# ZeayW/Multimodal-fusion-based-Pre-routing-Timing-Prediction-

Measured on AMD Instinct MI355X. Metric: train-step samples/sec, higher is better.
Workload: dtype bf16; 1 GPU; config B: 8 designs/step/GPU, 65536-node netlist, 64 levels, 256x256 tile, 1350 endpoints/design, UNet(max), bf16 operands / fp32 accumulate on the MFMA-bound contractions; U-Net activations and their gradients stored bf16, netlist tensors, statistics, parameters and gradients fp32; nodes=65536, levels=64, tile=256, endpoints_per_design=1350, cone_pruning=False, parallelism=dp1 (designs sharded, one all-reduce of the flat gradient per step), launch=one HIP graph replay per step (Adam inside)

## Files before the change

### multimodal-fusion-based-pre-routing-timing-prediction-_amd/csrc/linear.hip

```cpp
#include "gemm_engine.h"
#include <string.h>

namespace mmft {

static thread_local char g_err[512] = {0};

void set_error(const char* fmt, ...) {
  va_list ap;
  va_start(ap, fmt);
  vsnprintf(g_err, sizeof(g_err), fmt, ap);
  va_end(ap);
}

static int g_math_mode = 0;
int math_mode() { return __atomic_load_n(&g_math_mode, __ATOMIC_RELAXED); }

}
#include <mutex>
#include <string>
#include <vector>
#include <map>
namespace mmft {
struct ProfRec {
  const char* name;
// ... 256 lines not shown
    float v = x[i];
    if (act == ACT_RELU) v = v > 0.f ? v : 0.f;
    else if (act == ACT_LEAKY) v = v > 0.f ? v : v * slope;
    y[i] = v;
  }
}

__global__ void stamp_kernel(unsigned long long* slots, int index) { slots[index] = wall_clock64(); }

}

using namespace mmft;

extern "C" {

int mmft_version(void) { return 204; }

int mmft_set_math_mode(int mode) {
  MMFT_REQUIRE(mode == MMFT_MATH_F32 || mode == MMFT_MATH_BF16, "set_math_mode: unknown mode %d", mode);
  __atomic_store_n(&mmft::g_math_mode, mode, __ATOMIC_RELAXED);
  return MMFT_OK;
}

int mmft_get_math_mode(void) { return mmft::math_mode(); }

int mmft_prof_enable(int on) {
  std::lock_guard<std::mutex> lk(mmft::g_prof_mu);
  mmft::g_prof = on != 0;
  return MMFT_OK;
}

// ... 212 lines not shown
```

### multimodal-fusion-based-pre-routing-timing-prediction-_amd/csrc/unet16_conv.hip

```cpp
#include <type_traits>
#include "unet16.h"

namespace mmft {

struct U16PackDesc {
  const float* w;
  u16* out;
  int rows, K;
  int taps;
  int mode;
  int Rsrc, Ksrc;
};

__global__ void __launch_bounds__(256) u16_pack_kernel(const U16PackDesc* __restrict__ descs, long long* __restrict__ counters,
                                                       int ncounters, long long inc) {
  if (counters && blockIdx.x == 0 && blockIdx.y == 0 && (int)threadIdx.x < ncounters) counters[threadIdx.x] += inc;
  const U16PackDesc d = descs[blockIdx.y];
  const int mode = d.mode & 3, KW = (d.mode & 4) ? 8 : 4, G = KW / 4;
  const int KB = d.K / (4 * KW), MB = d.rows / 16;
  const long long items = (long long)MB * d.taps * KB * 64 * G;
  for (long long e = (long long)blockIdx.x * 256 + threadIdx.x; e < items; e += (long long)gridDim.x * 256) {
    const int g = (int)(e % G);
    const int lane = (int)((e / G) & 63);
    long long f = e / (64 * G);
// ... 462 lines not shown
  if (!name[0])
    snprintf(name, sizeof(name), EVAL ? "u16_conv3x3_eval_kernel<%d,%d,%dx%d%s>" : "u16_conv3x3_kernel<%d,%d,%dx%d%s>", RGB ? 3 : CI, COB,
             TH, TW, a.stats ? "" : "");
  MMFT_LAUNCH_LDS(name, flops, bytes, (u16_conv3x3_kernel<CI, COB, TH, TW, RGB, EVAL>), dim3(grid_x, a.CO / COB), dim3(256),
                  C::LDS_BYTES, st, a);
  return check_launch(EVAL ? "u16_conv3x3_eval" : "u16_conv3x3");
}

template <bool EVAL>
static int u16_conv_dispatch(U16ConvArgs& a, int rgb_f32, int Ci, hipStream_t st, double flops, double bytes) {
  int th, tw;
  u16_tile_shape(a.W, &th, &tw);
  a.tiles_x = (a.W + tw - 1) / tw;
  a.tiles_y = (a.H + th - 1) / th;
  a.tiles = a.N * a.tiles_x * a.tiles_y;
  const int cob = a.CO % 32 == 0 ? 32 : 16, gy = a.CO / cob;
  int cap = 2048 / gy;
  const int gx = a.tiles < cap ? a.tiles : cap;
#define U16_CONV(CIV, COBV, RGBV)                                                                           \
  (tw == 64 ? u16_conv_launch_t<CIV, COBV, 4, 64, RGBV, EVAL>(a, gx, st, flops, bytes)                      \
            : u16_conv_launch_t<CIV, COBV, 8, 32, RGBV, EVAL>(a, gx, st, flops, bytes))
  if (rgb_f32) return U16_CONV(16, 16, true);
  if (cob == 16) {
    if (Ci == 16) return U16_CONV(16, 16, false);
    if (Ci == 32) return U16_CONV(32, 16, false);
    if (Ci == 64) return U16_CONV(64, 16, false);
    return U16_CONV(128, 16, false);
  }
  if (Ci == 16) return U16_CONV(16, 32, false);
  if (Ci == 32) return U16_CONV(32, 32, false);
  if (Ci == 64) return U16_CONV(64, 32, false);
// ... 142 lines not shown
```

### multimodal-fusion-based-pre-routing-timing-prediction-_amd/csrc/unet16_ew.hip

```cpp
#include "unet16.h"

namespace mmft {

__device__ __forceinline__ double wave_sum_d(double v) {
  for (int o = 32; o > 0; o >>= 1) v += __shfl_xor(v, o, 64);
  return v;
}

__global__ void __launch_bounds__(64) u16_bn_finalize_kernel(const float* __restrict__ stats, int tiles_per_image, int N, int C,
                                                             double count, float eps, const float* __restrict__ gamma,
                                                             const float* __restrict__ beta, float* __restrict__ bnp) {
  const int img = blockIdx.x / C, c = blockIdx.x % C, lane = threadIdx.x;
  const long long NC = (long long)N * C;
  double s = 0.0, ss = 0.0;
  for (int t = lane; t < tiles_per_image; t += 64) {
    const float* p = stats + ((long long)(img * tiles_per_image + t) * 2) * C;
    s += (double)p[c];
    ss += (double)p[C + c];
  }
  s = wave_sum_d(s);
  ss = wave_sum_d(ss);
  if (lane == 0) {
    const double mean = s / count;
    double var = ss / count - mean * mean;
    if (var < 0.0) var = 0.0;
    const float invstd = (float)(1.0 / sqrt(var + (double)eps));
    const float scale = gamma[c] * invstd;
    const long long o = (long long)img * C + c;
    bnp[o] = (float)mean;
    bnp[NC + o] = invstd;
    bnp[2 * NC + o] = (float)var;
    bnp[3 * NC + o] = scale;
    bnp[4 * NC + o] = __fmaf_rn(-(float)mean, scale, beta[c]);
  }
}

struct U16Running {
  float* mean;
  float* var;
  float momentum;
  double count;
};
__device__ __forceinline__ void u16_running_update(const float* __restrict__ bnp, int N, int C, const U16Running& run) {
  const int c = threadIdx.x;
  if (c >= C) return;
  const long long NC = (long long)N * C;
  double rm = (double)run.mean[c], rv = (double)run.var[c];
  for (int img = 0; img < N; ++img) {
    const double var = (double)bnp[2 * NC + (long long)img * C + c];
// ... 5 lines not shown
  run.var[c] = (float)rv;
}

struct U16ApplyArgs {
  const u16* z;
  const float* scale;
  const float* shift;
  u16* a;
  int lda;
  u16* pooled;
  int N, H, W, C, pool_mode;
  const float* bnp;
  U16Running run;
};

__global__ void __launch_bounds__(256) u16_bn_apply_kernel(U16ApplyArgs p) {
  if (p.run.mean && blockIdx.x == 0) u16_running_update(p.bnp, p.N, p.C, p.run);
  const int CG = p.C / 8;
  const long long per_img = (long long)p.H * p.W * CG, total = per_img * p.N;
  for (long long it = (long long)blockIdx.x * 256 + threadIdx.x; it < total; it += (long long)gridDim.x * 256) {
    const int cg = (int)(it % CG);
    const long long pix = it / CG;
    const int img = (int)(it / per_img);
    float sc[8], sh[8], f[8];
    const float* s0 = p.scale + (long long)img * p.C + cg * 8;
    const float* h0 = p.shift + (long long)img * p.C + cg * 8;
    *reinterpret_cast<f32x4*>(sc) = *reinterpret_cast<const f32x4*>(s0);
    *reinterpret_cast<f32x4*>(sc + 4) = *reinterpret_cast<const f32x4*>(s0 + 4);
    *reinterpret_cast<f32x4*>(sh) = *reinterpret_cast<const f32x4*>(h0);
    *reinterpret_cast<f32x4*>(sh + 4) = *reinterpret_cast<const f32x4*>(h0 + 4);
    unpack8(*reinterpret_cast<const u32x4*>(p.z + pix * p.C + cg * 8), f);
#pragma unroll
    for (int j = 0; j < 8; ++j) {
      const float t = bn_pre(f[j], sc[j], sh[j]);
      f[j] = t > 0.f ? t : 0.f;
    }
    *reinterpret_cast<u32x4*>(p.a + pix * p.lda + cg * 8) = pack8(f);
  }
}

__global__ void __launch_bounds__(256) u16_bn_apply_pool_kernel(U16ApplyArgs p) {
  if (p.run.mean && blockIdx.x == 0) u16_running_update(p.bnp, p.N, p.C, p.run);
  const int CG = p.C / 8, H2 = p.H / 2, W2 = p.W / 2;
  const long long per_img = (long long)H2 * W2 * CG, total = per_img * p.N;
  for (long long it = (long long)blockIdx.x * 256 + threadIdx.x; it < total; it += (long long)gridDim.x * 256) {
    const int cg = (int)(it % CG);
    const long long win = it / CG;
    const int x2 = (int)(win % W2), y2 = (int)((win / W2) % H2), img = (int)(win / ((long long)W2 * H2));
    float sc[8], sh[8];
    const float* s0 = p.scale + (long long)img * p.C + cg * 8;
    const float* h0 = p.shift + (long long)img * p.C + cg * 8;
    *reinterpret_cast<f32x4*>(sc) = *reinterpret_cast<const f32x4*>(s0);
    *reinterpret_cast<f32x4*>(sc + 4) = *reinterpret_cast<const f32x4*>(s0 + 4);
    *reinterpret_cast<f32x4*>(sh) = *reinterpret_cast<const f32x4*>(h0);
    *reinterpret_cast<f32x4*>(sh + 4) = *reinterpret_cast<const f32x4*>(h0 + 4);
    const long long p00 = ((long long)img * p.H + 2 * y2) * p.W + 2 * x2;
    u32x4 zv[4];
#pragma unroll
    for (int k = 0; k < 4; ++k)
      zv[k] = *reinterpret_cast<const u32x4*>(p.z + (p00 + (k >> 1) * p.W + (k & 1)) * p.C + cg * 8);
    float best[8];
#pragma unroll
    for (int k = 0; k < 4; ++k) {
      float f[8];
      unpack8(zv[k], f);
#pragma unroll
      for (int j = 0; j < 8; ++j) {
        const float t = bn_pre(f[j], sc[j], sh[j]);
        f[j] = t > 0.f ? t : 0.f;
      }
      const u32x4 av = pack8(f);
      *reinterpret_cast<u32x4*>(p.a + (p00 + (k >> 1) * p.W + (k & 1)) * p.lda + cg * 8) = av;
      unpack8(av, f);
#pragma unroll
      for (int j = 0; j < 8; ++j) {
        if (p.pool_mode == MMFT_POOL_MAX) best[j] = (k == 0 || f[j] > best[j] || f[j] != f[j]) ? f[j] : best[j];
        else best[j] = k == 0 ? f[j] : best[j] + f[j];
      }
    }
    if (p.pool_mode != MMFT_POOL_MAX) {
#pragma unroll
      for (int j = 0; j < 8; ++j) best[j] *= 0.25f;
    }
    *reinterpret_cast<u32x4*>(p.pooled + (((long long)img * H2 + y2) * W2 + x2) * p.C + cg * 8) = pack8(best);
  }
}

__global__ void __launch_bounds__(256) u16_bn_bwd_partial_kernel(const u16* __restrict__ g, const u16* __restrict__ z,
                                                                 const float* __restrict__ bnp, long long rows, int N, int C,
                                                                 int blocks_per_image, float* __restrict__ partial) {
  __shared__ float red[2][256 * 8];
  const int img = blockIdx.x / blocks_per_image, blk = blockIdx.x % blocks_per_image;
  const long long NC = (long long)N * C;
  const long long rpb = (rows + blocks_per_image - 1) / blocks_per_image;
  const long long r0 = (long long)blk * rpb, r1 = r0 + rpb < rows ? r0 + rpb : rows;
  const int CG = C / 8;
  const int rstep = 256 / CG;
  const int cg = threadIdx.x % CG, rl = threadIdx.x / CG;
  float s[8], sx[8];
// ... 91 lines not shown
    const int cg = (int)(it % CG);
    const long long pix = it / CG;
    const int img = (int)(it / per_img);
    const long long o = (long long)img * C + cg * 8, e = pix * C + cg * 8;
    float gv[8], zf[8], out[8];
    unpack8(*reinterpret_cast<const u32x4*>(g + e), gv);
    unpack8(*reinterpret_cast<const u32x4*>(z + e), zf);
#pragma unroll
    for (int j = 0; j < 8; ++j) {
      const float mu = bnp[o + j], is = bnp[NC + o + j], sc = bnp[3 * NC + o + j], sh = bnp[4 * NC + o + j];
      const float gm = bn_pre(zf[j], sc, sh) > 0.f ? gv[j] : 0.f;
      const float xh = (zf[j] - mu) * is;
      out[j] = sc * (gm - coef[o + j] - xh * coef[NC + o + j]);
    }
    *reinterpret_cast<u32x4*>(dz + e) = pack8(out);
  }
}

struct U16PoolBwdArgs {
  const u16* a;
  int lda;
  const u16* gskip;
  int ldg;
  const u16* gp;
  u16* g;
  int N, H, W, C, pool_mode;
};

__global__ void __launch_bounds__(256) u16_pool_bwd_kernel(U16PoolBwdArgs p) {
  const int CG = p.C / 8, H2 = p.H / 2, W2 = p.W / 2;
// ... 68 lines not shown
  MMFT_REQUIRE(!running_mean == !running_var, "u16_bn_apply: running_mean and running_var come together");
  MMFT_REQUIRE(aligned16(z) && aligned16(a) && aligned16(bnp) && (!pooled || aligned16(pooled)), "u16_bn_apply: 16-byte alignment");
  DeviceGuard dg(device);
  const long long NC = (long long)N * C;
  U16ApplyArgs p{reinterpret_cast<const u16*>(z), bnp + 3 * NC, bnp + 4 * NC, reinterpret_cast<u16*>(a), lda,
                 reinterpret_cast<u16*>(pooled), N, H, W, C, pool_mode, bnp, U16Running{running_mean, running_var, momentum, (double)H * W}};
  const double by = 2.0 * N * H * W * C * (pooled ? 2.25 : 2.0);
  if (pooled) {
    const long long items = (long long)N * (H / 2) * (W / 2) * (C / 8);
    MMFT_LAUNCH("u16_bn_apply_pool_kernel", 0.0, by, u16_bn_apply_pool_kernel, dim3(ew_grid(items)), dim3(256), (hipStream_t)stream, p);
  } else {
    const long long items = (long long)N * H * W * (C / 8);
    MMFT_LAUNCH("u16_bn_apply_kernel", 0.0, by, u16_bn_apply_kernel, dim3(ew_grid(items)), dim3(256), (hipStream_t)stream, p);
  }
  return check_launch("u16_bn_apply");
}

long long mmft_u16_bn_bwd_workspace_bytes(int N, long long pixels_per_image, int C) {
  return (long long)N * u16_bwd_blocks(pixels_per_image) * 2 * C * 4 + (long long)2 * N * C * 4;
}

int mmft_u16_bn_bwd(const void* g, const void* z, const float* bnp, void* dz, float* dgamma, float* dbeta, int accumulate, int N,
                    long long pixels_per_image, int C, float* workspace, long long workspace_bytes, int device, void* stream) {
  MMFT_REQUIRE(g && z && bnp && dz && dgamma && dbeta && N > 0 && pixels_per_image > 0 && C >= 8 && C % 8 == 0 && C <= 128,
               "u16_bn_bwd: bad arguments (C a multiple of 8, <= 128)");
  MMFT_REQUIRE(workspace && workspace_bytes >= mmft_u16_bn_bwd_workspace_bytes(N, pixels_per_image, C), "u16_bn_bwd: workspace too small");
  MMFT_REQUIRE(aligned16(g) && aligned16(z) && aligned16(dz), "u16_bn_bwd: 16-byte alignment");
  DeviceGuard dg(device);
  hipStream_t st = (hipStream_t)stream;
  const int bpi = u16_bwd_blocks(pixels_per_image);
// ... 2 lines not shown
  const double elems = (double)N * pixels_per_image * C;
  MMFT_LAUNCH("u16_bn_bwd_partial_kernel", 0.0, 4.0 * elems, u16_bn_bwd_partial_kernel, dim3(N * bpi), dim3(256), st,
              reinterpret_cast<const u16*>(g), reinterpret_cast<const u16*>(z), bnp, pixels_per_image, N, C, bpi, partial);
  int rc = check_launch("u16_bn_bwd_partial");
  if (rc) return rc;
  MMFT_LAUNCH("u16_bn_bwd_finalize_kernel", 0.0, 8.0 * N * bpi * C, u16_bn_bwd_finalize_kernel, dim3(C), dim3(256), st, partial, bpi, N, C,
              (double)pixels_per_image, coef, dgamma, dbeta, accumulate ? 1 : 0);
  rc = check_launch("u16_bn_bwd_finalize");
  if (rc) return rc;
  const long long items = (long long)N * pixels_per_image * (C / 8);
  MMFT_LAUNCH("u16_bn_bwd_apply_kernel", 0.0, 6.0 * elems, u16_bn_bwd_apply_kernel, dim3(ew_grid(items)), dim3(256), st,
              reinterpret_cast<const u16*>(g), reinterpret_cast<const u16*>(z), bnp, coef, reinterpret_cast<u16*>(dz), pixels_per_image, N, C);
  return check_launch("u16_bn_bwd_apply");
}

int mmft_u16_pool_bwd(const void* a, int lda, const void* gskip, int ldg, const void* gp, void* g, int N, int H, int W, int C,
                      int pool_mode, int device, void* stream) {
  MMFT_REQUIRE(a && gp && g && N > 0 && H > 0 && W > 0 && H % 2 == 0 && W % 2 == 0 && C >= 8 && C % 8 == 0 && lda >= C && lda % 8 == 0 &&
                   (!gskip || (ldg >= C && ldg % 8 == 0)),
               "u16_pool_bwd: bad arguments");
  MMFT_REQUIRE(aligned16(a) && aligned16(gp) && aligned16(g) && (!gskip || aligned16(gskip)), "u16_pool_bwd: 16-byte alignment");
  DeviceGuard dg(device);
  U16PoolBwdArgs p{reinterpret_cast<const u16*>(a), lda, reinterpret_cast<const u16*>(gskip), ldg, reinterpret_cast<const u16*>(gp),
                   reinterpret_cast<u16*>(g), N, H, W, C, pool_mode};
  const long long items = (long long)N * (H / 2) * (W / 2) * (C / 8);
  MMFT_LAUNCH("u16_pool_bwd_kernel", 0.0, 2.0 * N * H * W * C * (gskip ? 3.25 : 2.25), u16_pool_bwd_kernel, dim3(ew_grid(items)), dim3(256),
              (hipStream_t)stream, p);
  return check_launch("u16_pool_bwd");
}

// ... 2 lines not shown
```

### multimodal-fusion-based-pre-routing-timing-prediction-_amd/mmft/lib.py

```python
import contextlib
import ctypes
import os
import re
import threading
import torch

_HERE = os.path.dirname(os.path.abspath(__file__))
PKG_DIR = os.path.dirname(_HERE)
LIB_PATH = os.environ.get('MMFT_LIB') or os.path.join(PKG_DIR, 'lib', 'libmmft_hip.so')
HEADER_PATH = os.path.join(os.path.dirname(PKG_DIR), 'include', 'mmft.h')
EXT_HEADER_PATH = os.path.join(os.path.dirname(PKG_DIR), 'include', 'mmft_report.h')
PLACE_HEADER_PATH = os.path.join(os.path.dirname(PKG_DIR), 'include', 'mmft_place.h')
INCR_HEADER_PATH = os.path.join(os.path.dirname(PKG_DIR), 'include', 'mmft_incr.h')

_lib = None


def _parse_header(path):
    with open(path) as f:
        text = f.read()
    text = re.sub(r'/\*.*?\*/', '', text, flags=re.S)
    decls = {}
    for ret, name, params in re.findall(r'\b(int|long long|const char\*)\s+(mmft_[a-z0-9_]+)\s*\(([^)]*)\)\s*;', text):
        args = []
        params = params.strip()
        if params and params != 'void':
            for prm in params.split(','):
                prm = prm.strip()
# ... 20 lines not shown
    return _parse_header(HEADER_PATH)


def ext_decls():
    return _parse_header(EXT_HEADER_PATH)


def place_decls():
    return _parse_header(PLACE_HEADER_PATH)


def incr_decls():
    return _parse_header(INCR_HEADER_PATH)


def header_symbols():
    return sorted(header_decls())


def load():
    global _lib
    if _lib is None:
        if not os.path.exists(LIB_PATH):
            raise RuntimeError(
                f"libmmft_hip.so not found at {LIB_PATH}; build it with `python __graft_entry__.py build` "
                f"(make -C {os.path.join(PKG_DIR, 'csrc')}). There is no CPU/eager fallback for the hot path.")
        _lib = ctypes.CDLL(LIB_PATH)
        for name, (res, args) in header_decls().items():
            fn = getattr(_lib, name)
            fn.restype = res
# ... 76 lines not shown
    return int(rc)


_INCR = {}


def incr(name, *args):
    fn = _INCR.get(name)
    if fn is None:
        decls = incr_decls()
        if name not in decls:
            raise RuntimeError(f'{name} is not declared in {INCR_HEADER_PATH}')
        fn = getattr(load(), name)
        fn.restype, fn.argtypes = decls[name]
        _INCR[name] = fn
    rc = fn(*[a.data_ptr() if isinstance(a, _Tensor) else a for a in args])
    if rc != 0:
        raise RuntimeError(f"{name} failed ({rc}): {load().mmft_last_error().decode()}")
    return int(rc)


_workspace = {}
_retired = []
_scope = threading.local()


@contextlib.contextmanager
def scratch_owner(owner):
    prev, _scope.owner = getattr(_scope, 'owner', None), owner
    try:
# ... 108 lines not shown
```

### multimodal-fusion-based-pre-routing-timing-prediction-_amd/mmft/unet16.py

```python
import ctypes
import functools
import math
import weakref

import torch
from torch import nn

from . import gradsink, lib, ops

ENABLED = True


def supported(net, x, frozen_stats=False):
    if not ENABLED or net.bilinear or x.dim() != 4 or x.shape[1] != 3 or x.dtype != torch.float32 or not x.is_cuda:
        return False
    if x.shape[0] > 1 and not net.inc.per_sample_stats and not frozen_stats:
        return False
    H, W = x.shape[2], x.shape[3]
    return H % 8 == 0 and W % 32 == 0 and H >= 8


def _params(net):
    ps = net.__dict__.get('_u16_param_list')
    if ps is None:
# ... 162 lines not shown

@functools.lru_cache(maxsize=16)
def _bwd_sizes(N, H, W):
    lv, P = _geometry(N, H, W)
    sizes = [('g%d' % i, P[_CONV[i][2]] * _CONV[i][1]) for i in range(1, 15)] + [('dz%d' % i, P[_CONV[i][2]] * _CONV[i][1]) for i in range(1, 15)]
    sizes += [('gcat3', P[0] * 32), ('gcat2', P[1] * 64), ('gcat1', P[2] * 128), ('gp1', P[1] * 16), ('gp2', P[2] * 32), ('gp3', P[3] * 64)]
    q = lib.query
    ws_bytes = max([q('mmft_u16_outconv_bwd_workspace_bytes', N, H, W)] +
                   [q('mmft_u16_bn_bwd_workspace_bytes', N, lv[_CONV[i][2]][0] * lv[_CONV[i][2]][1], _CONV[i][1]) for i in range(1, 15)] +
                   [q('mmft_u16_conv3x3_wgrad_workspace_bytes', N, lv[_CONV[i][2]][0], lv[_CONV[i][2]][1], _CONV[i][0], _CONV[i][1])
                    for i in range(1, 15)] +
                   [q('mmft_u16_convt_wgrad_workspace_bytes', N, lv[u[4]][0], lv[u[4]][1], u[0]) for u in _UP.values()])
    return sizes, ws_bytes


BATCH_REDUCE = True


@functools.lru_cache(maxsize=16)
def _slab_sizes(N, H, W):
    lv, _ = _geometry(N, H, W)
    q = lib.query
    sizes = [('sw%d' % i, q('mmft_u16_conv3x3_wgrad_workspace_bytes', N, lv[_CONV[i][2]][0], lv[_CONV[i][2]][1], _CONV[i][0], _CONV[i][1]) // 4)
             for i in range(1, 15)]
    sizes += [('st%d' % k, q('mmft_u16_convt_wgrad_workspace_bytes', N, lv[u[4]][0], lv[u[4]][1], u[0]) // 4) for k, u in _UP.items()]
    sizes += [('so', q('mmft_u16_outconv_bwd_workspace_bytes', N, H, W) // 4)]
    return sizes


def _run_forward(net, xn, pool_mode, packs, T, F, out, geom):
    N, H, W = geom
    dev, st = lib.stream_args(out)
    lv, _ = _geometry(N, H, W)
    convs = _layers(net)
    ups = [net.up1.up, net.up2.up, net.up3.up]
    packs.refresh(net, counters=net._batch_counters(), inc=N if net.inc.per_sample_stats else 1)
    per_img = ctypes.c_int(0)
    for i in range(1, 15):
        Ci, Co, l, inp = _CONV[i]
        h, w = lv[l]
        cv, bn = convs[i - 1]
        xin = xn if inp == 'x' else T[inp]
        lib.load().mmft_u16_conv_tiles(N, h, w, ctypes.byref(per_img))
        lib.call('mmft_u16_conv3x3', xin, 1 if inp == 'x' else 0, packs.ptr('f%d' % (i - 1)), T['z%d' % i], F['stats'], N, h, w,
                 Ci, Co, dev, st)
        lib.call('mmft_u16_bn_finalize', F['stats'], per_img.value, N, Co, h * w, float(bn.eps), bn.weight.detach(), bn.bias.detach(),
                 F['bnp%d' % i], dev, st)
        abuf_name, lda, pooled = _ACT[i]
        lib.call('mmft_u16_bn_apply', T['z%d' % i], F['bnp%d' % i], T[abuf_name], lda, T[pooled] if pooled else None, N, h, w, Co,
                 pool_mode, float(bn.momentum), bn.running_mean, bn.running_var, dev, st)
        for k, (uCi, uin, cat, coff, ul) in _UP.items():
            if uin == abuf_name:
                up = ups[k]
                uh, uw = lv[ul]
                lib.call('mmft_u16_convt_fwd', T[uin], packs.ptr('tf%d' % k), up.bias.detach() if up.bias is not None else None,
                         T[cat].data_ptr() + coff * 2, 2 * (uCi // 2), N, uh, uw, uCi, dev, st)
    oc = net.outc.conv[0]
    lib.call('mmft_u16_outconv_fwd', T['a14'], oc.weight.detach(), oc.bias.detach() if oc.bias is not None else None, out, N, H, W,
             pool_mode, dev, st)


@functools.lru_cache(maxsize=16)
def _eval_sizes(N, H, W):
    return [(name, n) for name, n in _fwd_sizes(N, H, W)[0] if not name.startswith('z')]

# ... 82 lines not shown
        so = SL['so']
        lib.call('mmft_u16_outconv_bwd', T['a14'], oc.weight.detach(), oc.bias.detach() if oc.bias is not None else None, g, G['g14'],
                 None, None, 0, N, H, W, pool_mode, so, so.numel() * 4, dev, st)
        ns = lib.query('mmft_u16_outconv_bwd_slabs', N, H, W)
        reduce_later(so.data_ptr(), s_w.out, ns, 17, 16, 1, s_w.accumulate)
        if s_b is not None:
            reduce_later(so.data_ptr() + 64, s_b.out, ns, 17, 1, 1, s_b.accumulate)

    def conv_backward(i):
        Ci, Co, l, inp = _CONV[i]
        h, w = lv[l]
        cv, bn = convs[i - 1]
        s_g, s_bt = sinks[id(bn.weight)], sinks[id(bn.bias)]
        if s_g.accumulate != s_bt.accumulate:
            raise RuntimeError('unet16: BatchNorm weight / bias sinks out of step')
        lib.call('mmft_u16_bn_bwd', G['g%d' % i], T['z%d' % i], F['bnp%d' % i], G['dz%d' % i], s_g.out, s_bt.out, int(s_g.accumulate),
                 N, h * w, Co, ws, ws.numel() * 4, dev, st)
        s_cw = sinks[id(cv.weight)]
        xin = xn if inp == 'x' else T[inp]
        if SL is None:
            lib.call('mmft_u16_conv3x3_wgrad', xin, 1 if inp == 'x' else 0, G['dz%d' % i], s_cw.out, int(s_cw.accumulate), N, h, w, Ci, Co,
                     ws, ws.numel() * 4, dev, st)
        else:
            sw = SL['sw%d' % i]
            lib.call('mmft_u16_conv3x3_wgrad', xin, 1 if inp == 'x' else 0, G['dz%d' % i], None, 0, N, h, w, Ci, Co,
                     sw, sw.numel() * 4, dev, st)
            reduce_later(sw.data_ptr(), s_cw.out, lib.query('mmft_u16_conv3x3_wgrad_slabs', N, h, w, Ci, Co), Co * 9 * Ci, Co * 9 * Ci, 1,
                         s_cw.accumulate)
        if inp == 'x':
            return
        tgt = {'cat1': 'gcat1', 'cat2': 'gcat2', 'cat3': 'gcat3', 'p1': 'gp1', 'p2': 'gp2', 'p3': 'gp3'}.get(inp)
        if tgt is None:
# ... 20 lines not shown
            if s_ub is not None:
                reduce_later(stb.data_ptr() + 4 * wel, s_ub.out, ns, wel + 4 * Co, Co, 4, s_ub.accumulate)
        lib.call('mmft_u16_convt_dgrad', gslice, 2 * Co, packs.ptr('tb%d' % k), G[g_target], N, uh, uw, uCi, dev, st)

    def pool_backward(cat, C, l, gp, g_target):
        h, w = lv[l]
        lib.call('mmft_u16_pool_bwd', T[cat], 2 * C, G['g' + cat], 2 * C, G[gp], G[g_target], N, h, w, C, pool_mode, dev, st)

    conv_backward(14); conv_backward(13); up_backward(2, 'g12')
    conv_backward(12); conv_backward(11); up_backward(1, 'g10')
    conv_backward(10); conv_backward(9); up_backward(0, 'g8')
    conv_backward(8); conv_backward(7); pool_backward('cat1', 64, 2, 'gp3', 'g6')
    conv_backward(6); conv_backward(5); pool_backward('cat2', 32, 1, 'gp2', 'g4')
    conv_backward(4); conv_backward(3); pool_backward('cat3', 16, 0, 'gp1', 'g2')
    conv_backward(2); conv_backward(1)
    if table:
        lib.call('mmft_slab_reduce_batch', torch.tensor(table, dtype=torch.int64), len(table), dev, st)


REPLAY = True


class _Token:
    __slots__ = ('__weakref__',)


class _Replay:

    def __init__(self, key):
        self.key, self.x_ref, self.x_version = key, None, None
        self.fwd, self.bwd = lib.GraphReplay(), lib.GraphReplay()
        self.pending = None
# ... 92 lines not shown
```

Before: 2441 designs/s.

## Fuse BN finalize with apply for small U-Net levels and add fused BN backward

Adds a single-launch kernel that recomputes the per-image BatchNorm coefficients from tile statistics inside each apply block and writes bnp and running stats from block 0. It is used for small spatial levels with at least 64 channels, removing a separate finalize launch and its dependency bubble. It also adds a fused BN backward kernel (disabled by default), switches the conv dispatch to 16-channel output blocks when the 128-input-channel grid is too small, and chunks the slab-reduce batch. The cost is redundant coefficient recomputation per block and some added code paths.

```diff
diff --git a/include/mmft_unet_small.h b/include/mmft_unet_small.h
--- /dev/null
+++ b/include/mmft_unet_small.h
@@ -0,0 +1,19 @@
+#ifndef MMFT_UNET_SMALL_H
+#define MMFT_UNET_SMALL_H
+
+#include "mmft.h"
+
+#ifdef __cplusplus
+extern "C" {
+#endif
+
+int mmft_u16_bn_finalize_apply(const float* stats, int tiles_per_image, int N, int C, long long pixels_per_image, float eps,
+                               const float* gamma, const float* beta, float* bnp, const void* z, void* a, int lda, void* pooled, int H,
+                               int W, int pool_mode, float momentum, float* running_mean, float* running_var, int device, void* stream);
+int mmft_u16_bn_bwd_fused(const void* g, const void* z, const float* bnp, void* dz, float* sums, float* dgamma, float* dbeta,
+                          int accumulate, int N, long long pixels_per_image, int C, int device, void* stream);
+
+#ifdef __cplusplus
+}
+#endif
+#endif
diff --git a/multimodal-fusion-based-pre-routing-timing-prediction-_amd/csrc/linear.hip b/multimodal-fusion-based-pre-routing-timing-prediction-_amd/csrc/linear.hip
--- a/multimodal-fusion-based-pre-routing-timing-prediction-_amd/csrc/linear.hip
+++ b/multimodal-fusion-based-pre-routing-timing-prediction-_amd/csrc/linear.hip
@@ -294,7 +294,7 @@
 
 extern "C" {
 
-int mmft_version(void) { return 204; }
+int mmft_version(void) { return 205; }
 
 int mmft_set_math_mode(int mode) {
   MMFT_REQUIRE(mode == MMFT_MATH_F32 || mode == MMFT_MATH_BF16, "set_math_mode: unknown mode %d", mode);
diff --git a/multimodal-fusion-based-pre-routing-timing-prediction-_amd/csrc/unet16_conv.hip b/multimodal-fusion-based-pre-routing-timing-prediction-_amd/csrc/unet16_conv.hip
--- a/multimodal-fusion-based-pre-routing-timing-prediction-_amd/csrc/unet16_conv.hip
+++ b/multimodal-fusion-based-pre-routing-timing-prediction-_amd/csrc/unet16_conv.hip
@@ -500,7 +500,8 @@
   a.tiles_x = (a.W + tw - 1) / tw;
   a.tiles_y = (a.H + th - 1) / th;
   a.tiles = a.N * a.tiles_x * a.tiles_y;
-  const int cob = a.CO % 32 == 0 ? 32 : 16, gy = a.CO / cob;
+  const bool narrow = Ci == 128 && (long long)a.tiles * (a.CO / 32) < 256;
+  const int cob = (a.CO % 32 == 0 && !narrow) ? 32 : 16, gy = a.CO / cob;
   int cap = 2048 / gy;
   const int gx = a.tiles < cap ? a.tiles : cap;
 #define U16_CONV(CIV, COBV, RGBV)                                                                           \
diff --git a/multimodal-fusion-based-pre-routing-timing-prediction-_amd/csrc/unet16_ew.hip b/multimodal-fusion-based-pre-routing-timing-prediction-_amd/csrc/unet16_ew.hip
--- a/multimodal-fusion-based-pre-routing-timing-prediction-_amd/csrc/unet16_ew.hip
+++ b/multimodal-fusion-based-pre-routing-timing-prediction-_amd/csrc/unet16_ew.hip
@@ -1,10 +1,34 @@
 #include "unet16.h"
+#include "../../include/mmft_unet_small.h"
 
 namespace mmft {
 
 __device__ __forceinline__ double wave_sum_d(double v) {
   for (int o = 32; o > 0; o >>= 1) v += __shfl_xor(v, o, 64);
   return v;
+}
+
+struct U16Coef {
+  float mean, invstd, var, scale, shift;
+};
+__device__ __forceinline__ U16Coef u16_bn_coef(double s, double ss, double count, float eps, float gamma, float beta) {
+  const double mean = s / count;
+  double var = ss / count - mean * mean;
+  if (var < 0.0) var = 0.0;
+  U16Coef k;
+  k.invstd = (float)(1.0 / sqrt(var + (double)eps));
+  k.scale = gamma * k.invstd;
+  k.mean = (float)mean;
+  k.var = (float)var;
+  k.shift = __fmaf_rn(-(float)mean, k.scale, beta);
+  return k;
+}
+__device__ __forceinline__ void u16_bn_store_coef(const U16Coef& k, float* __restrict__ bnp, long long NC, long long o) {
+  bnp[o] = k.mean;
+  bnp[NC + o] = k.invstd;
+  bnp[2 * NC + o] = k.var;
+  bnp[3 * NC + o] = k.scale;
+  bnp[4 * NC + o] = k.shift;
 }
 
 __global__ void __launch_bounds__(64) u16_bn_finalize_kernel(const float* __restrict__ stats, int tiles_per_image, int N, int C,
@@ -20,19 +44,7 @@
   }
   s = wave_sum_d(s);
   ss = wave_sum_d(ss);
-  if (lane == 0) {
-    const double mean = s / count;
-    double var = ss / count - mean * mean;
-    if (var < 0.0) var = 0.0;
-    const float invstd = (float)(1.0 / sqrt(var + (double)eps));
-    const float scale = gamma[c] * invstd;
-    const long long o = (long long)img * C + c;
-    bnp[o] = (float)mean;
-    bnp[NC + o] = invstd;
-    bnp[2 * NC + o] = (float)var;
-    bnp[3 * NC + o] = scale;
-    bnp[4 * NC + o] = __fmaf_rn(-(float)mean, scale, beta[c]);
-  }
+  if (lane == 0) u16_bn_store_coef(u16_bn_coef(s, ss, count, eps, gamma[c], beta[c]), bnp, NC, (long long)img * C + c);
 }
 
 struct U16Running {
@@ -68,28 +80,68 @@
   U16Running run;
 };
 
+__device__ __forceinline__ void u16_load_coef8(const float* __restrict__ s0, const float* __restrict__ h0, float sc[8], float sh[8]) {
+  *reinterpret_cast<f32x4*>(sc) = *reinterpret_cast<const f32x4*>(s0);
+  *reinterpret_cast<f32x4*>(sc + 4) = *reinterpret_cast<const f32x4*>(s0 + 4);
+  *reinterpret_cast<f32x4*>(sh) = *reinterpret_cast<const f32x4*>(h0);
+  *reinterpret_cast<f32x4*>(sh + 4) = *reinterpret_cast<const f32x4*>(h0 + 4);
+}
+
+__device__ __forceinline__ void u16_apply_item(const U16ApplyArgs& p, long long pix, int cg, const float sc[8], const float sh[8]) {
+  float f[8];
+  unpack8(*reinterpret_cast<const u32x4*>(p.z + pix * p.C + cg * 8), f);
+#pragma unroll
+  for (int j = 0; j < 8; ++j) {
+    const float t = bn_pre(f[j], sc[j], sh[j]);
+    f[j] = t > 0.f ? t : 0.f;
+  }
+  *reinterpret_cast<u32x4*>(p.a + pix * p.lda + cg * 8) = pack8(f);
+}
+
+__device__ __forceinline__ void u16_apply_pool_item(const U16ApplyArgs& p, int img, int y2, int x2, int cg, const float sc[8],
+                                                    const float sh[8]) {
+  const int H2 = p.H / 2, W2 = p.W / 2;
+  const long long p00 = ((long long)img * p.H + 2 * y2) * p.W + 2 * x2;
+  u32x4 zv[4];
+#pragma unroll
+  for (int k = 0; k < 4; ++k)
+    zv[k] = *reinterpret_cast<const u32x4*>(p.z + (p00 + (k >> 1) * p.W + (k & 1)) * p.C + cg * 8);
+  float best[8];
+#pragma unroll
+  for (int k = 0; k < 4; ++k) {
+    float f[8];
+    unpack8(zv[k], f);
+#pragma unroll
+    for (int j = 0; j < 8; ++j) {
+      const float t = bn_pre(f[j], sc[j], sh[j]);
+      f[j] = t > 0.f ? t : 0.f;
+    }
+    const u32x4 av = pack8(f);
+    *reinterpret_cast<u32x4*>(p.a + (p00 + (k >> 1) * p.W + (k & 1)) * p.lda + cg * 8) = av;
+    unpack8(av, f);
+#pragma unroll
+    for (int j = 0; j < 8; ++j) {
+      if (p.pool_mode == MMFT_POOL_MAX) best[j] = (k == 0 || f[j] > best[j] || f[j] != f[j]) ? f[j] : best[j];
+      else best[j] = k == 0 ? f[j] : best[j] + f[j];
+    }
+  }
+  if (p.pool_mode != MMFT_POOL_MAX) {
+#pragma unroll
+    for (int j = 0; j < 8; ++j) best[j] *= 0.25f;
+  }
+  *reinterpret_cast<u32x4*>(p.pooled + (((long long)img * H2 + y2) * W2 + x2) * p.C + cg * 8) = pack8(best);
+}
+
 __global__ void __launch_bounds__(256) u16_bn_apply_kernel(U16ApplyArgs p) {
   if (p.run.mean && blockIdx.x == 0) u16_running_update(p.bnp, p.N, p.C, p.run);
   const int CG = p.C / 8;
   const long long per_img = (long long)p.H * p.W * CG, total = per_img * p.N;
   for (long long it = (long long)blockIdx.x * 256 + threadIdx.x; it < total; it += (long long)gridDim.x * 256) {
     const int cg = (int)(it % CG);
-    const long long pix = it / CG;
     const int img = (int)(it / per_img);
-    float sc[8], sh[8], f[8];
-    const float* s0 = p.scale + (long long)img * p.C + cg * 8;
-    const float* h0 = p.shift + (long long)img * p.C + cg * 8;
-    *reinterpret_cast<f32x4*>(sc) = *reinterpret_cast<const f32x4*>(s0);
-    *reinterpret_cast<f32x4*>(sc + 4) = *reinterpret_cast<const f32x4*>(s0 + 4);
-    *reinterpret_cast<f32x4*>(sh) = *reinterpret_cast<const f32x4*>(h0);
-    *reinterpret_cast<f32x4*>(sh + 4) = *reinterpret_cast<const f32x4*>(h0 + 4);
-    unpack8(*reinterpret_cast<const u32x4*>(p.z + pix * p.C + cg * 8), f);
-#pragma unroll
-    for (int j = 0; j < 8; ++j) {
-      const float t = bn_pre(f[j], sc[j], sh[j]);
-      f[j] = t > 0.f ? t : 0.f;
-    }
-    *reinterpret_cast<u32x4*>(p.a + pix * p.lda + cg * 8) = pack8(f);
+    float sc[8], sh[8];
+    u16_load_coef8(p.scale + (long long)img * p.C + cg * 8, p.shift + (long long)img * p.C + cg * 8, sc, sh);
+    u16_apply_item(p, it / CG, cg, sc, sh);
   }
 }
 
@@ -102,41 +154,75 @@
     const long long win = it / CG;
     const int x2 = (int)(win % W2), y2 = (int)((win / W2) % H2), img = (int)(win / ((long long)W2 * H2));
     float sc[8], sh[8];
-    const float* s0 = p.scale + (long long)img * p.C + cg * 8;
-    const float* h0 = p.shift + (long long)img * p.C + cg * 8;
-    *reinterpret_cast<f32x4*>(sc) = *reinterpret_cast<const f32x4*>(s0);
-    *reinterpret_cast<f32x4*>(sc + 4) = *reinterpret_cast<const f32x4*>(s0 + 4);
-    *reinterpret_cast<f32x4*>(sh) = *reinterpret_cast<const f32x4*>(h0);
-    *reinterpret_cast<f32x4*>(sh + 4) = *reinterpret_cast<const f32x4*>(h0 + 4);
-    const long long p00 = ((long long)img * p.H + 2 * y2) * p.W + 2 * x2;
-    u32x4 zv[4];
-#pragma unroll
-    for (int k = 0; k < 4; ++k)
-      zv[k] = *reinterpret_cast<const u32x4*>(p.z + (p00 + (k >> 1) * p.W + (k & 1)) * p.C + cg * 8);
-    float best[8];
-#pragma unroll
-    for (int k = 0; k < 4; ++k) {
-      float f[8];
-      unpack8(zv[k], f);
-#pragma unroll
-      for (int j = 0; j < 8; ++j) {
-        const float t = bn_pre(f[j], sc[j], sh[j]);
-        f[j] = t > 0.f ? t : 0.f;
-      }
-      const u32x4 av = pack8(f);
-      *reinterpret_cast<u32x4*>(p.a + (p00 + (k >> 1) * p.W + (k & 1)) * p.lda + cg * 8) = av;
-      unpack8(av, f);
-#pragma unroll
-      for (int j = 0; j < 8; ++j) {
-        if (p.pool_mode == MMFT_POOL_MAX) best[j] = (k == 0 || f[j] > best[j] || f[j] != f[j]) ? f[j] : best[j];
-        else best[j] = k == 0 ? f[j] : best[j] + f[j];
-      }
-    }
-    if (p.pool_mode != MMFT_POOL_MAX) {
-#pragma unroll
-      for (int j = 0; j < 8; ++j) best[j] *= 0.25f;
-    }
-    *reinterpret_cast<u32x4*>(p.pooled + (((long long)img * H2 + y2) * W2 + x2) * p.C + cg * 8) = pack8(best);
+    u16_load_coef8(p.scale + (long long)img * p.C + cg * 8, p.shift + (long long)img * p.C + cg * 8, sc, sh);
+    u16_apply_pool_item(p, img, y2, x2, cg, sc, sh);
+  }
+}
+
+struct U16FinArgs {
+  const float* stats;
+  int tiles_per_image;
+  float eps;
+  const float* gamma;
+  const float* beta;
+  float* bnp;
+  int blocks_per_image;
+};
+
+__device__ __forceinline__ U16Coef u16_coef_from_tiles(const U16FinArgs& f, int img, int C, int c, double count) {
+  double s[16], ss[16];
+#pragma unroll
+  for (int t = 0; t < 16; ++t) {
+    s[t] = ss[t] = 0.0;
+    if (t < f.tiles_per_image) {
+      const float* p = f.stats + ((long long)(img * f.tiles_per_image + t) * 2) * C;
+      s[t] += (double)p[c];
+      ss[t] += (double)p[C + c];
+    }
+  }
+#pragma unroll
+  for (int o = 8; o > 0; o >>= 1) {
+#pragma unroll
+    for (int t = 0; t < o; ++t) {
+      s[t] += s[t + o];
+      ss[t] += ss[t + o];
+    }
+  }
+  return u16_bn_coef(s[0], ss[0], count, f.eps, f.gamma[c], f.beta[c]);
+}
+
+template <bool POOL>
+__global__ void __launch_bounds__(256) u16_bn_finalize_apply_kernel(U16ApplyArgs p, U16FinArgs f) {
+  __shared__ __attribute__((aligned(16))) float coef[2][256];
+  const int tid = threadIdx.x, C = p.C;
+  if (blockIdx.x == 0) {
+    const int slots = 256 / C, c = tid % C;
+    if (tid < slots * C)
+      for (int img = tid / C; img < p.N; img += slots)
+        u16_bn_store_coef(u16_coef_from_tiles(f, img, C, c, p.run.count), f.bnp, (long long)p.N * C, (long long)img * C + c);
+    __syncthreads();
+    if (p.run.mean) u16_running_update(f.bnp, p.N, C, p.run);
+    return;
+  }
+  const int b = (int)blockIdx.x - 1, img = b / f.blocks_per_image, blk = b % f.blocks_per_image;
+  if (tid < C) {
+    const U16Coef k = u16_coef_from_tiles(f, img, C, tid, p.run.count);
+    coef[0][tid] = k.scale;
+    coef[1][tid] = k.shift;
+  }
+  __syncthreads();
+  const int CG = C / 8;
+  const int per_img = (POOL ? (p.H / 2) * (p.W / 2) : p.H * p.W) * CG;
+  for (int it = blk * 256 + tid; it < per_img; it += f.blocks_per_image * 256) {
+    const int cg = it % CG, q = it / CG;
+    float sc[8], sh[8];
+#pragma unroll
+    for (int j = 0; j < 8; ++j) {
+      sc[j] = coef[0][cg * 8 + j];
+      sh[j] = coef[1][cg * 8 + j];
+    }
+    if (POOL) u16_apply_pool_item(p, img, q / (p.W / 2), q % (p.W / 2), cg, sc, sh);
+    else u16_apply_item(p, (long long)img * p.H * p.W + q, cg, sc, sh);
   }
 }
 
@@ -258,6 +344,97 @@
       out[j] = sc * (gm - coef[o + j] - xh * coef[NC + o + j]);
     }
     *reinterpret_cast<u32x4*>(dz + e) = pack8(out);
+  }
+}
+
+template <int THREADS>
+__global__ void __launch_bounds__(THREADS) u16_bn_bwd_fused_kernel(const u16* __restrict__ g, const u16* __restrict__ z,
+                                                                   const float* __restrict__ bnp, u16* __restrict__ dz,
+                                                                   float* __restrict__ sums, int P, int N, int C) {
+  constexpr int ITEMS = 4, PARTS = THREADS / 16;
+  __shared__ float red[THREADS][9];
+  __shared__ double part[2][PARTS][8];
+  __shared__ float cf[16];
+  const int CG = C / 8, img = blockIdx.x / CG, cg = blockIdx.x % CG, tid = threadIdx.x;
+  const long long NC = (long long)N * C, o = (long long)img * C + cg * 8, base = (long long)img * P;
+  float mu[8], is[8], sc[8], sh[8];
+#pragma unroll
+  for (int j = 0; j < 8; ++j) {
+    mu[j] = bnp[o + j];
+    is[j] = bnp[NC + o + j];
+    sc[j] = bnp[3 * NC + o + j];
+    sh[j] = bnp[4 * NC + o + j];
+  }
+  u32x4 gq[ITEMS], zq[ITEMS];
+#pragma unroll
+  for (int k = 0; k < ITEMS; ++k) {
+    const int pix = k * THREADS + tid;
+    gq[k] = zq[k] = u32x4{0u, 0u, 0u, 0u};
+    if (pix < P) {
+      const long long e = (base + pix) * C + cg * 8;
+      gq[k] = *reinterpret_cast<const u32x4*>(g + e);
+      zq[k] = *reinterpret_cast<const u32x4*>(z + e);
+    }
+  }
+  float s[2][8];
+#pragma unroll
+  for (int j = 0; j < 8; ++j) s[0][j] = s[1][j] = 0.f;
+#pragma unroll
+  for (int k = 0; k < ITEMS; ++k) {
+    float gv[8], zf[8];
+    unpack8(gq[k], gv);
+    unpack8(zq[k], zf);
+#pragma unroll
+    for (int j = 0; j < 8; ++j) {
+      const float gm = bn_pre(zf[j], sc[j], sh[j]) > 0.f ? gv[j] : 0.f;
+      s[0][j] += gm;
+      s[1][j] = __fmaf_rn(gm, (zf[j] - mu[j]) * is[j], s[1][j]);
+    }
+  }
+#pragma unroll
+  for (int which = 0; which < 2; ++which) {
+#pragma unroll
+    for (int j = 0; j < 8; ++j) red[tid][j] = s[which][j];
+    __syncthreads();
+    if (tid < THREADS / 2) {
+      const int v = tid & 7, q = tid >> 3;
+      double a = 0.0;
+#pragma unroll
+      for (int i = 0; i < 16; ++i) a += (double)red[q * 16 + i][v];
+      part[which][q][v] = a;
+    }
+    __syncthreads();
+  }
+  if (tid < 16) {
+    const int which = tid >> 3, v = tid & 7;
+    double a = 0.0;
+#pragma unroll 8
+    for (int q = 0; q < PARTS; ++q) a += part[which][q][v];
+    cf[tid] = (float)(a / (double)P);
+    sums[((long long)img * 2 + which) * C + cg * 8 + v] = (float)a;
+  }
+  __syncthreads();
+  float c0[8], c1[8];
+#pragma unroll
+  for (int j = 0; j < 8; ++j) {
+    c0[j] = cf[j];
+    c1[j] = cf[8 + j];
+  }
+#pragma unroll
+  for (int k = 0; k < ITEMS; ++k) {
+    const int pix = k * THREADS + tid;
+    if (pix < P) {
+      float gv[8], zf[8], out[8];
+      unpack8(gq[k], gv);
+      unpack8(zq[k], zf);
+#pragma unroll
+      for (int j = 0; j < 8; ++j) {
+        const float gm = bn_pre(zf[j], sc[j], sh[j]) > 0.f ? gv[j] : 0.f;
+        const float xh = (zf[j] - mu[j]) * is[j];
+        out[j] = sc[j] * (gm - c0[j] - xh * c1[j]);
+      }
+      *reinterpret_cast<u32x4*>(dz + (base + pix) * C + cg * 8) = pack8(out);
+    }
   }
 }
 
@@ -356,6 +533,37 @@
     MMFT_LAUNCH("u16_bn_apply_kernel", 0.0, by, u16_bn_apply_kernel, dim3(ew_grid(items)), dim3(256), (hipStream_t)stream, p);
   }
   return check_launch("u16_bn_apply");
+}
+
+int mmft_u16_bn_finalize_apply(const float* stats, int tiles_per_image, int N, int C, long long pixels_per_image, float eps,
+                               const float* gamma, const float* beta, float* bnp, const void* z, void* a, int lda, void* pooled, int H,
+                               int W, int pool_mode, float momentum, float* running_mean, float* running_var, int device, void* stream) {
+  MMFT_REQUIRE(stats && gamma && beta && bnp && z && a && N > 0 && H > 0 && W > 0 && C >= 8 && C % 8 == 0 && C <= 256 && lda >= C &&
+                   lda % 8 == 0 && pixels_per_image == (long long)H * W,
+               "u16_bn_finalize_apply: bad arguments");
+  MMFT_REQUIRE(tiles_per_image > 0 && tiles_per_image <= 16, "u16_bn_finalize_apply: 1 .. 16 tiles per image (got %d)", tiles_per_image);
+  MMFT_REQUIRE(pixels_per_image <= 16 * 256, "u16_bn_finalize_apply: at most 4096 pixels per image");
+  MMFT_REQUIRE(!pooled || (H % 2 == 0 && W % 2 == 0), "u16_bn_finalize_apply: pooling needs even H, W");
+  MMFT_REQUIRE(!running_mean == !running_var, "u16_bn_finalize_apply: running_mean and running_var come together");
+  MMFT_REQUIRE(aligned16(z) && aligned16(a) && (!pooled || aligned16(pooled)), "u16_bn_finalize_apply: 16-byte alignment");
+  DeviceGuard dg(device);
+  U16ApplyArgs p{reinterpret_cast<const u16*>(z), nullptr, nullptr, reinterpret_cast<u16*>(a), lda, reinterpret_cast<u16*>(pooled),
+                 N, H, W, C, pool_mode, bnp, U16Running{running_mean, running_var, momentum, (double)pixels_per_image}};
+  const long long items = (pooled ? (long long)(H / 2) * (W / 2) : (long long)H * W) * (C / 8);
+  int bpi = 1;
+  for (int ipt = 4; ipt >= 1; ipt >>= 1) {
+    bpi = cdiv(items, 256 * ipt);
+    if ((long long)N * bpi >= 256) break;
+  }
+  U16FinArgs f{stats, tiles_per_image, eps, gamma, beta, bnp, bpi};
+  const double by = 2.0 * N * H * W * C * (pooled ? 2.25 : 2.0) + 8.0 * N * tiles_per_image * C * (bpi + 1.0) + 20.0 * N * C;
+  if (pooled)
+    MMFT_LAUNCH("u16_bn_finalize_apply_kernel<pool>", 0.0, by, u16_bn_finalize_apply_kernel<true>, dim3(1 + N * bpi), dim3(256),
+                (hipStream_t)stream, p, f);
+  else
+    MMFT_LAUNCH("u16_bn_finalize_apply_kernel", 0.0, by, u16_bn_finalize_apply_kernel<false>, dim3(1 + N * bpi), dim3(256),
+                (hipStream_t)stream, p, f);
+  return check_launch("u16_bn_finalize_apply");
 }
 
 long long mmft_u16_bn_bwd_workspace_bytes(int N, long long pixels_per_image, int C) {
@@ -388,6 +596,31 @@
   return check_launch("u16_bn_bwd_apply");
 }
 
+int mmft_u16_bn_bwd_fused(const void* g, const void* z, const float* bnp, void* dz, float* sums, float* dgamma, float* dbeta,
+                          int accumulate, int N, long long pixels_per_image, int C, int device, void* stream) {
+  MMFT_REQUIRE(g && z && bnp && dz && sums && N > 0 && pixels_per_image > 0 && C >= 8 && C % 8 == 0 && C <= 128,
+               "u16_bn_bwd_fused: bad arguments (C a multiple of 8, <= 128)");
+  MMFT_REQUIRE(pixels_per_image <= 4096, "u16_bn_bwd_fused: at most 4096 pixels per image (got %lld)", pixels_per_image);
+  MMFT_REQUIRE(!dgamma == !dbeta, "u16_bn_bwd_fused: dgamma and dbeta come together");
+  MMFT_REQUIRE(aligned16(g) && aligned16(z) && aligned16(dz), "u16_bn_bwd_fused: 16-byte alignment");
+  DeviceGuard dg(device);
+  hipStream_t st = (hipStream_t)stream;
+  const int P = (int)pixels_per_image;
+  const double by = 6.0 * N * (double)P * C + 8.0 * N * C;
+  const u16 *gp = reinterpret_cast<const u16*>(g), *zp = reinterpret_cast<const u16*>(z);
+  if (P <= 1024)
+    MMFT_LAUNCH("u16_bn_bwd_fused_kernel<256>", 0.0, by, u16_bn_bwd_fused_kernel<256>, dim3(N * (C / 8)), dim3(256), st, gp, zp, bnp,
+                reinterpret_cast<u16*>(dz), sums, P, N, C);
+  else
+    MMFT_LAUNCH("u16_bn_bwd_fused_kernel<1024>", 0.0, by, u16_bn_bwd_fused_kernel<1024>, dim3(N * (C / 8)), dim3(1024), st, gp, zp, bnp,
+                reinterpret_cast<u16*>(dz), sums, P, N, C);
+  int rc = check_launch("u16_bn_bwd_fused");
+  if (rc || !dgamma) return rc;
+  rc = launch_slab_reduce_strided(sums, N, 2LL * C, C, dbeta, accumulate, st);
+  if (rc) return rc;
+  return launch_slab_reduce_strided(sums + C, N, 2LL * C, C, dgamma, accumulate, st);
+}
+
 int mmft_u16_pool_bwd(const void* a, int lda, const void* gskip, int ldg, const void* gp, void* g, int N, int H, int W, int C,
                       int pool_mode, int device, void* stream) {
   MMFT_REQUIRE(a && gp && g && N > 0 && H > 0 && W > 0 && H % 2 == 0 && W % 2 == 0 && C >= 8 && C % 8 == 0 && lda >= C && lda % 8 == 0 &&
diff --git a/multimodal-fusion-based-pre-routing-timing-prediction-_amd/mmft/lib.py b/multimodal-fusion-based-pre-routing-timing-prediction-_amd/mmft/lib.py
--- a/multimodal-fusion-based-pre-routing-timing-prediction-_amd/mmft/lib.py
+++ b/multimodal-fusion-based-pre-routing-timing-prediction-_amd/mmft/lib.py
@@ -12,6 +12,7 @@
 EXT_HEADER_PATH = os.path.join(os.path.dirname(PKG_DIR), 'include', 'mmft_report.h')
 PLACE_HEADER_PATH = os.path.join(os.path.dirname(PKG_DIR), 'include', 'mmft_place.h')
 INCR_HEADER_PATH = os.path.join(os.path.dirname(PKG_DIR), 'include', 'mmft_incr.h')
+SMALL_HEADER_PATH = os.path.join(os.path.dirname(PKG_DIR), 'include', 'mmft_unet_small.h')
 
 _lib = None
 
@@ -62,6 +63,10 @@
     return _parse_header(INCR_HEADER_PATH)
 
 
+def small_decls():
+    return _parse_header(SMALL_HEADER_PATH)
+
+
 def header_symbols():
     return sorted(header_decls())
 
@@ -168,6 +173,24 @@
         fn = getattr(load(), name)
         fn.restype, fn.argtypes = decls[name]
         _INCR[name] = fn
+    rc = fn(*[a.data_ptr() if isinstance(a, _Tensor) else a for a in args])
+    if rc != 0:
+        raise RuntimeError(f"{name} failed ({rc}): {load().mmft_last_error().decode()}")
+    return int(rc)
+
+
+_SMALL = {}
+
+
+def small(name, *args):
+    fn = _SMALL.get(name)
+    if fn is None:
+        decls = small_decls()
+        if name not in decls:
+            raise RuntimeError(f'{name} is not declared in {SMALL_HEADER_PATH}')
+        fn = getattr(load(), name)
+        fn.restype, fn.argtypes = decls[name]
+        _SMALL[name] = fn
     rc = fn(*[a.data_ptr() if isinstance(a, _Tensor) else a for a in args])
     if rc != 0:
         raise RuntimeError(f"{name} failed ({rc}): {load().mmft_last_error().decode()}")
diff --git a/multimodal-fusion-based-pre-routing-timing-prediction-_amd/mmft/unet16.py b/multimodal-fusion-based-pre-routing-timing-prediction-_amd/mmft/unet16.py
--- a/multimodal-fusion-based-pre-routing-timing-prediction-_amd/mmft/unet16.py
+++ b/multimodal-fusion-based-pre-routing-timing-prediction-_amd/mmft/unet16.py
@@ -200,7 +200,13 @@
     return sizes, ws_bytes
 
 
+SMALL_BN = True
+FUSED_FWD_MAX_TILES = 16
+FUSED_BWD_MAX_PIXELS = 1024
+SMALL_BN_BACKWARD = False
+FUSED_MIN_CHANNELS = 64
 BATCH_REDUCE = True
+SLAB_BATCH_MAX = 24
 
 
 @functools.lru_cache(maxsize=16)
@@ -211,7 +217,34 @@
              for i in range(1, 15)]
     sizes += [('st%d' % k, q('mmft_u16_convt_wgrad_workspace_bytes', N, lv[u[4]][0], lv[u[4]][1], u[0]) // 4) for k, u in _UP.items()]
     sizes += [('so', q('mmft_u16_outconv_bwd_workspace_bytes', N, H, W) // 4)]
+    sizes += [('sb%d' % i, N * 2 * _CONV[i][1]) for i in range(1, 15)]
     return sizes
+
+
+def bn_forward(stats, tiles_per_image, z, bnp, a, lda, pooled, N, h, w, C, pool_mode, eps, gamma, beta, momentum, running_mean,
+               running_var, dev, st):
+    if SMALL_BN and tiles_per_image <= FUSED_FWD_MAX_TILES and C >= FUSED_MIN_CHANNELS:
+        lib.small('mmft_u16_bn_finalize_apply', stats, tiles_per_image, N, C, h * w, eps, gamma, beta, bnp, z, a, lda, pooled, h, w,
+                 pool_mode, momentum, running_mean, running_var, dev, st)
+        return
+    lib.call('mmft_u16_bn_finalize', stats, tiles_per_image, N, C, h * w, eps, gamma, beta, bnp, dev, st)
+    lib.call('mmft_u16_bn_apply', z, bnp, a, lda, pooled, N, h, w, C, pool_mode, momentum, running_mean, running_var, dev, st)
+
+
+def bn_backward_fused(pixels_per_image, C):
+    return SMALL_BN and SMALL_BN_BACKWARD and pixels_per_image <= FUSED_BWD_MAX_PIXELS and C >= FUSED_MIN_CHANNELS
+
+
+def bn_backward(g, z, bnp, dz, dgamma, dbeta, accumulate, N, pixels_per_image, C, ws, dev, st, sums=None):
+    if not bn_backward_fused(pixels_per_image, C):
+        lib.call('mmft_u16_bn_bwd', g, z, bnp, dz, dgamma, dbeta, int(accumulate), N, pixels_per_image, C, ws, ws.numel() * 4, dev, st)
+        return []
+    if sums is None:
+        lib.small('mmft_u16_bn_bwd_fused', g, z, bnp, dz, ws, dgamma, dbeta, int(accumulate), N, pixels_per_image, C, dev, st)
+        return []
+    lib.small('mmft_u16_bn_bwd_fused', g, z, bnp, dz, sums, None, None, 0, N, pixels_per_image, C, dev, st)
+    return [[sums.data_ptr(), dbeta.data_ptr(), N, 2 * C, C, 1, int(accumulate)],
+            [sums.data_ptr() + 4 * C, dgamma.data_ptr(), N, 2 * C, C, 1, int(accumulate)]]
 
 
 def _run_forward(net, xn, pool_mode, packs, T, F, out, geom):
@@ -230,11 +263,10 @@
         lib.load().mmft_u16_conv_tiles(N, h, w, ctypes.byref(per_img))
         lib.call('mmft_u16_conv3x3', xin, 1 if inp == 'x' else 0, packs.ptr('f%d' % (i - 1)), T['z%d' % i], F['stats'], N, h, w,
                  Ci, Co, dev, st)
-        lib.call('mmft_u16_bn_finalize', F['stats'], per_img.value, N, Co, h * w, float(bn.eps), bn.weight.detach(), bn.bias.detach(),
-                 F['bnp%d' % i], dev, st)
         abuf_name, lda, pooled = _ACT[i]
-        lib.call('mmft_u16_bn_apply', T['z%d' % i], F['bnp%d' % i], T[abuf_name], lda, T[pooled] if pooled else None, N, h, w, Co,
-                 pool_mode, float(bn.momentum), bn.running_mean, bn.running_var, dev, st)
+        bn_forward(F['stats'], per_img.value, T['z%d' % i], F['bnp%d' % i], T[abuf_name], lda, T[pooled] if pooled else None, N, h, w, Co,
+                   pool_mode, float(bn.eps), bn.weight.detach(), bn.bias.detach(), float(bn.momentum), bn.running_mean, bn.running_var,
+                   dev, st)
         for k, (uCi, uin, cat, coff, ul) in _UP.items():
             if uin == abuf_name:
                 up = ups[k]
@@ -347,8 +379,8 @@
         s_g, s_bt = sinks[id(bn.weight)], sinks[id(bn.bias)]
         if s_g.accumulate != s_bt.accumulate:
             raise RuntimeError('unet16: BatchNorm weight / bias sinks out of step')
-        lib.call('mmft_u16_bn_bwd', G['g%d' % i], T['z%d' % i], F['bnp%d' % i], G['dz%d' % i], s_g.out, s_bt.out, int(s_g.accumulate),
-                 N, h * w, Co, ws, ws.numel() * 4, dev, st)
+        table.extend(bn_backward(G['g%d' % i], T['z%d' % i], F['bnp%d' % i], G['dz%d' % i], s_g.out, s_bt.out, s_g.accumulate, N, h * w, Co,
+                                 ws, dev, st, sums=SL.get('sb%d' % i) if SL is not None else None))
         s_cw = sinks[id(cv.weight)]
         xin = xn if inp == 'x' else T[inp]
         if SL is None:
@@ -399,8 +431,9 @@
     conv_backward(6); conv_backward(5); pool_backward('cat2', 32, 1, 'gp2', 'g4')
     conv_backward(4); conv_backward(3); pool_backward('cat3', 16, 0, 'gp1', 'g2')
     conv_backward(2); conv_backward(1)
-    if table:
-        lib.call('mmft_slab_reduce_batch', torch.tensor(table, dtype=torch.int64), len(table), dev, st)
+    for k in range(0, len(table), SLAB_BATCH_MAX):
+        rows = table[k:k + SLAB_BATCH_MAX]
+        lib.call('mmft_slab_reduce_batch', torch.tensor(rows, dtype=torch.int64), len(rows), dev, st)
 
 
 REPLAY = True
```

New measurement: 2464 designs/s, median of 6. About the same (+0.9%).
